# hmakelin/gisnav

Measured on AMD Instinct MI355X. Metric: matched frame-pairs/sec + PnP poses/sec, 640x480 cam-vs-tile, higher is better.
Workload: dtype f32-accurate FFN / out-projection / match-head GEMMs (each f32 operand split into 2 fp16 terms = 22 significant bits, 3 fp16 MFMA partial products, f32 accumulate; fp16-range guard active); attention INPUT projections (q, k, v: 18 of 66 launches) on 2 partial products -- the fp16 high term of the ac

## Files before the change

### gisnav_amd/csrc/gn_api.hip

```cpp
#include "gn_common.h"

#include <cstdio>
#include <cstring>
#include <cmath>
#include <cctype>
#include <algorithm>
#include <tuple>

using namespace gn;

namespace {

thread_local std::string g_err;

struct Linear { float* w = nullptr; float* b = nullptr; int out = 0, in = 0; uint16_t* wp = nullptr; float acc_scale = 1.f;
                uint16_t* wf = nullptr; int frag_order = -1;
                uint16_t* wf2 = nullptr;
                uint16_t* wfn = nullptr; };

struct Block {
  Linear proj_in;
  Linear proj_out;
  Linear ffn0;
  float* ln_g = nullptr; float* ln_b = nullptr;
// ... 93 lines not shown
  float *colbest = nullptr, *col2 = nullptr;
  bool cal_cols = false;
  int precision_api = 0;
  int feature = 0;
  int ransac_iters = 10; float ransac_reproj = 8.0f; double ransac_conf = 0.99;
  gn::PnpArgs last_pnp; bool last_pnp_valid = false; const int32_t* last_npts = nullptr;
  int dist_on = 0; double dist[5] = {0, 0, 0, 0, 0};
  float size_q[2] = {0.f, 0.f}, size_r[2] = {0.f, 0.f};
  int npad_run = 0;
  int n_layers = kMaxLayers;
  float threshold = 0.5f;
  std::string err;
  Linear input_proj;
  float* wr = nullptr;
  Block self_blk[kMaxLayers], cross_blk[kMaxLayers];
  Linear final_proj[kMaxLayers], matchability[kMaxLayers];
  std::map<std::string, bool> loaded;
  std::vector<std::string> required;
  float *desc = nullptr, *cos_t = nullptr, *sin_t = nullptr, *extent = nullptr;
  int32_t* nvalid = nullptr;
  float *x = nullptr, *qkv = nullptr, *ctx = nullptr, *msg = nullptr, *h = nullptr, *md = nullptr, *ls = nullptr;
  uint16_t *desc_p = nullptr, *x_p = nullptr, *ctx_p = nullptr, *msg_p = nullptr, *h_p = nullptr, *md_p = nullptr;
  size_t Tmax = 0;
  int planes_mode = 0;
  float* sim = nullptr;
  uint16_t *qkb = nullptr, *vtb = nullptr;
  float* attn_part = nullptr; unsigned int* attn_tickets = nullptr;
  int attn_split = 1;
  int attn_variant = 4;
  int stop_after = 0;
  int launch_count = 0;
  int no_planes = 0;
  int dbg_planes = 0;
  uint16_t* dbg_wp = nullptr; size_t dbg_wp_n = 0;
  int dbg_out = 0;
  uint16_t* dbg_yp = nullptr; size_t dbg_yp_n = 0;
  int dbg_vt_skip = 0;
  int dbg_reuse = 0;
  uint16_t* dbg_ap = nullptr; size_t dbg_ap_n = 0;
  int gemm_variant = -1;
  float *rowmax = nullptr, *rowlog = nullptr, *colmax = nullptr, *collog = nullptr, *max0 = nullptr;
  int32_t *m0 = nullptr, *m1 = nullptr;
  float *cpart_m = nullptr, *cpart_s = nullptr;
  int32_t* cpart_i = nullptr;
  float* rot4 = nullptr;
  float *rpart_a = nullptr, *rpart_b = nullptr;
  unsigned int* tickets = nullptr;
  int64_t* e_idx = nullptr; float* e_score = nullptr; float* e_mkp = nullptr; float* e_obj = nullptr;
  int defer_join = 0, sub_last_B = 0, sub_last_np = 0;
  int sub_serial = 0;
  int cu_mask_mode = 0;
  int use_lists = 1;
  int ncu = 256;
  int fused_proj_status = -1;
  bool fused_proj_pending = true;
  int fused_proj_off = 0;
  int qkv_in_tail = 1;
  int skinny = 1;
  int auto_level = 3; float cert_eps_lvl[2] = {-1.f, -1.f}; long long auto_pairs = 0, auto_wide = 0, auto_narrow = 0, auto_calls_lvl[2] = {0, 0}, auto_switches = 0;
  int ffn_products = 3;
  int qkv_products = 2;
  unsigned long long* tile_feedback = nullptr;
  int* lists = nullptr; long long lists_stride = 0;
  int n_sub = 1; hipStream_t sub_s[8] = {}; hipEvent_t ev_fork = nullptr; hipEvent_t ev_join[8] = {}; bool sub_pending[8] = {};
  int overlap = 0; unsigned long long calls = 0;
  hipStream_t s_pnp = nullptr; hipEvent_t ev_gather[2][8] = {}, ev_pnp[2][8] = {}; bool pnp_pending[2][8] = {}, pnp_recorded[2][8] = {};
  hipEvent_t ev_head[8] = {};
  float* o_mkp[2] = {nullptr, nullptr}; float* o_obj[2] = {nullptr, nullptr}; int32_t* o_nmatch[2] = {nullptr, nullptr};
  int prep_fused = 1;
  int sift_h = 0, sift_w = 0; std::vector<void*> sift_allocs; SiftPyramid sift_py; float* sift_tmp = nullptr;
  float* sift_dk = nullptr; std::vector<std::vector<float>> sift_kernels; std::vector<int> sift_koff;
  int4* sift_cand = nullptr; int* sift_counts = nullptr; SiftKeypoint* sift_kp = nullptr;
  int sift_max_cand = 0, sift_max_kp = 0, sift_raw_cap = 0, sift_batch = 0; long long sift_kp_stride = 0;
  std::vector<int32_t> sift_totals;
  struct SpConv { float* wf = nullptr; float* b = nullptr; int cout = 0, cin = 0, taps = 0, cout_pad = 0; bool have_w = false, have_b = false;
                  uint16_t* wfh = nullptr; float acc_scale = 1.f; };
  SpConv sp[12];
  std::vector<void*> sp_allocs; int sp_h = 0, sp_w = 0, sp_chunk = 0, sp_cap = 0, sp_max = 0;
  float *sp_x = nullptr, *sp_y = nullptr, *sp_z = nullptr, *sp_maps[6] = {};
  int *sp_cand = nullptr, *sp_counts = nullptr, *sp_index = nullptr;
  float* vo_norm2 = nullptr; int32_t* vo_nn_idx = nullptr; float* vo_nn_dist = nullptr; uint8_t* vo_good = nullptr;
  uint8_t* mask_ws = nullptr;
  float* pts_ws = nullptr;
  gn::HypResult* hyp_ws = nullptr;
  uint8_t* rmask_ws = nullptr;
  gn::RansacState *rstate_ws = nullptr, *rstate_base = nullptr;
  std::vector<void*> allocs;
  std::vector<void*> ws_allocs;
  bool timing = false;
  hipEvent_t ev[2 * 128];
  int ev_stage[128]; int n_ev = 0; bool ev_ready = false;
  float stage_ms[ST_COUNT] = {0};
  bool ktiming = false;
  std::vector<hipEvent_t> kev;
  std::vector<double> kflops;
  std::vector<double> kbytes;
  std::vector<int> kclass;
  std::vector<const char*> kname;
  size_t kused = 0;
};

namespace {

#define GN_HIP(call)                                                                              \
  do {                                                                                            \
    hipError_t e_ = (call);                                                                       \
// ... 362 lines not shown
    StageTimer tm(c, s, ST_PREP);
    PrepArgs p;
    p.desc_q = v.desc_q; p.kpt_q = v.kpt_q; p.n_q = v.n_q; p.stride_q = v.stride_q;
    p.desc_r = v.desc_r; p.kpt_r = v.kpt_r; p.n_r = v.n_r; p.stride_r = v.stride_r;
    p.kpt_format = v.kpt_format; p.B = B; p.npad = np; p.wr = c->wr;
    p.desc = c->desc; p.kxy = nullptr; p.cos_t = c->cos_t; p.sin_t = c->sin_t; p.nvalid = c->nvalid; p.extent = c->extent;
    p.size_q[0] = c->size_q[0]; p.size_q[1] = c->size_q[1]; p.size_r[0] = c->size_r[0]; p.size_r[1] = c->size_r[1];
    p.feature = c->feature; p.x = nullptr; p.xp = nullptr;
    p.ovf_clear = (c->planes_mode && c->guard) ? c->ovf : nullptr;
    p.ovf_init = (c->dbg_trip_group && c->ovf == c->ovf_base + (c->dbg_trip_group - 1)) ? 1u : 0u;
    p.desc_p = nullptr; p.rot4 = nullptr; p.rot_stride = (long long)c->Tmax;
    const bool planes_only = c->planes_mode && c->x_planes_only && c->n_layers > 0;
    if (c->feature == 1) {
      p.x = planes_only ? nullptr : c->x; p.xp = c->planes_mode ? c->x_p : nullptr;
      launch_prep(p, s);
      if (c->rot4 && c->qkv_fused) launch_rot_table(c->cos_t, c->sin_t, c->rot4, T, (long long)c->Tmax, s);
    } else {
      const bool rot = c->rot4 && c->qkv_fused, split = c->planes_mode != 0;
      if (c->prep_fused) { p.rot4 = rot ? c->rot4 : nullptr; p.desc_p = split ? c->desc_p : nullptr; }
      launch_prep(p, s);
      if (rot && !p.rot4) launch_rot_table(c->cos_t, c->sin_t, c->rot4, T, (long long)c->Tmax, s);
      if (split && !p.desc_p) launch_split_hm16(c->desc, c->desc_p, T, kInDim, 1.0f, s);
      GemmArgs g = gemm_args(c->desc, kInDim, c->input_proj, c->x, kDim, T);
      g.drop_f32 = planes_only ? 1 : 0;
      gemm(c, EPI_BIAS, g, s);
    }
  }
  if (c->use_lists && c->lists) {
    const int g = (int)(c->ovf - c->ovf_base);
    launch_tile_lists(c->nvalid, BS, np, c->lists, (c->tile_feedback && g >= 0 && g < 8) ? c->tile_feedback + g : nullptr, s);
  }
  bool qkv_done = false;
  for (int i = 0; i < c->n_layers; ++i) {
    {
      const Block& blk = c->self_blk[i];
      if (!qkv_done) {
        StageTimer tm(c, s, ST_PROJ);
        GemmArgs g = gemm_args(c->x, kDim, blk.proj_in, c->qkv, 3 * kDim, T);
        g.cos_t = c->cos_t; g.sin_t = c->sin_t; g.rot_cols = 2 * kDim;
        if (bf16v2 && qkv_projection(c, blk, false, T, np, vt_perm, s)) {
        } else if (bf16v2) {
          g.Yb = c->qkb; g.ldyb = 2 * kDim; g.Vt = c->vtb; g.vt_start = 2 * kDim; g.q_cols = kDim; g.qscale = 0.125f; g.npad = np; g.vt_perm = vt_perm; g.half_fmt = c->attn_f16;
          gemm(c, EPI_ROTARY_BF16, g, s);
        } else {
          gemm(c, EPI_ROTARY, g, s);
        }
      }
      {
        StageTimer tm(c, s, ST_ATTN);
        AttnArgs a; a.ovf = nullptr;
        a.q = c->qkv; a.ldq = 3 * kDim; a.k = c->qkv + kDim; a.ldk = 3 * kDim; a.v = c->qkv + 2 * kDim; a.ldv = 3 * kDim;
        a.out = c->ctx; a.ldo = kDim; a.nvalid = c->nvalid; a.npad = np; a.cross = 0; a.qscale = 0.125f; a.BS = BS;
        a.outp = attn_planes ? c->ctx_p : nullptr; a.ovf = (attn_planes && c->guard) ? c->ovf : nullptr;
        a.qb = c->qkb; a.ldqb = 2 * kDim; a.kb = c->qkb + kDim; a.ldkb = 2 * kDim; a.vt = c->vtb; a.half_fmt = c->attn_f16; a.tiles = (c->use_lists && c->lists) ? c->lists : nullptr; a.ncu = c->ncu;
        if (bf16v2) attn_split(c, a);
        timed_attention(c, a, bf16v2, s);
        if (c->planes_mode && !attn_planes) launch_split_hm16(c->ctx, c->ctx_p, T, kDim, 1.0f, s);
      }
      if (!tail_folds_out_proj(c, blk, T)) {
        StageTimer tm(c, s, ST_PROJ);
        GemmArgs g = gemm_args(c->ctx, kDim, blk.proj_out, c->msg, kDim, T);
        gemm(c, EPI_BIAS, g, s);
      }
      { StageTimer tm(c, s, ST_FFN); qkv_done = ffn(c, blk, T, s, false, bf16v2 ? &c->cross_blk[i] : nullptr, true, np, vt_perm); }
    }
    {
      const Block& blk = c->cross_blk[i];
      if (!qkv_done) {
        StageTimer tm(c, s, ST_PROJ);
        GemmArgs g = gemm_args(c->x, kDim, blk.proj_in, c->qkv, 2 * kDim, T);
        g.scale = 0.35355339059327373f;
        g.scale_cols = kDim;
        if (bf16v2 && qkv_projection(c, blk, true, T, np, vt_perm, s)) {
        } else if (bf16v2) {
          g.Yb = c->qkb; g.ldyb = kDim; g.Vt = c->vtb; g.vt_start = kDim; g.q_cols = 0; g.qscale = 1.0f; g.npad = np; g.vt_perm = vt_perm; g.half_fmt = c->attn_f16;
          gemm(c, EPI_SCALE_BF16, g, s);
        } else {
          gemm(c, EPI_SCALE_COLS, g, s);
        }
      }
      {
        StageTimer tm(c, s, ST_ATTN);
        AttnArgs a; a.ovf = nullptr;
        a.q = c->qkv; a.ldq = 2 * kDim; a.k = c->qkv; a.ldk = 2 * kDim; a.v = c->qkv + kDim; a.ldv = 2 * kDim;
        a.out = c->ctx; a.ldo = kDim; a.nvalid = c->nvalid; a.npad = np; a.cross = 1; a.qscale = 1.0f; a.BS = BS;
        a.outp = attn_planes ? c->ctx_p : nullptr; a.ovf = (attn_planes && c->guard) ? c->ovf : nullptr;
        a.qb = c->qkb; a.ldqb = kDim; a.kb = c->qkb; a.ldkb = kDim; a.vt = c->vtb; a.half_fmt = c->attn_f16; a.tiles = (c->use_lists && c->lists) ? c->lists : nullptr; a.ncu = c->ncu;
        if (bf16v2) attn_split(c, a);
        timed_attention(c, a, bf16v2, s);
        if (c->planes_mode && !attn_planes) launch_split_hm16(c->ctx, c->ctx_p, T, kDim, 1.0f, s);
      }
      if (!tail_folds_out_proj(c, blk, T)) {
        StageTimer tm(c, s, ST_PROJ);
        GemmArgs g = gemm_args(c->ctx, kDim, blk.proj_out, c->msg, kDim, T);
        gemm(c, EPI_BIAS, g, s);
      }
      { StageTimer tm(c, s, ST_FFN); qkv_done = ffn(c, blk, T, s, i == c->n_layers - 1, (bf16v2 && i + 1 < c->n_layers) ? &c->self_blk[i + 1] : nullptr, false, np, vt_perm); }
    }
  }
  {
    StageTimer tm(c, s, ST_HEAD);
    const int li = c->n_layers - 1;
    GemmArgs g = gemm_args(c->x, kDim, c->final_proj[li], c->md, kDim, T);
    g.scale = 0.25f; g.scale_cols = kDim;
    gemm(c, EPI_SCALE_COLS, g, s);
    launch_matchability(c->x, c->matchability[li].w, c->matchability[li].b, c->ls, T, s);
    HeadArgs hd;
    hd.sim = c->sim; hd.ls = c->ls; hd.nvalid = c->nvalid; hd.B = B; hd.npad = np; hd.threshold = c->threshold;
    hd.rowmax = c->rowmax; hd.rowlog = c->rowlog; hd.colmax = c->colmax; hd.collog = c->collog;
    hd.m0 = c->m0; hd.max0 = c->max0; hd.m1 = c->m1;
    hd.ovf = (c->planes_mode && c->guard) ? c->ovf : nullptr;
    hd.max0b = c->max0b; hd.rpart_c = c->rpart_c; hd.uncert = c->certify ? c->uncert : nullptr;
    hd.cert_eps = (c->precision == GN_PREC_F32) ? c->cert_eps_f32 : cert_eps_now(c);
    if (hd.uncert && c->precision != GN_PREC_F32 && ffn_auto(c)) { hd.uncert_alt = c->uncert_alt; hd.cert_eps_alt = c->cert_eps_lvl[3 - c->auto_level]; }
    hd.idx = v.idx; hd.score = v.score; hd.n_match = v.n_match; hd.kmax = c->npad;
    hd.md = c->planes_mode ? (const void*)c->md_p : (const void*)c->md; hd.md_f32 = c->planes_mode ? 0 : 1;
    hd.cpart_m = c->cpart_m; hd.cpart_s = c->cpart_s; hd.cpart_i = c->cpart_i; hd.rpart_a = c->rpart_a; hd.rpart_b = c->rpart_b; hd.tickets = c->tickets;
    hd.dbg_ts = (c->head_stamps && c->sim) ? reinterpret_cast<long long*>(c->sim) : nullptr;
    if (c->cal_cols) { hd.colbest = c->colbest; hd.col2 = c->col2; }
    if (c->head_fused || !c->sim) {
      timed_launch(c, s, 0, 2.0 * 2.0 * B * (double)np * np * kDim,
                   2.0 * (4.0 * T * kDim) + 4.0 * T * 4.0 + 8.0 * B * np * 3.0,
                   "k_head_fused (2 sweeps)", [&] { launch_match_head_fused(hd, s); });
      return GN_OK;
    }
    GemmArgs gs;
    memset(&gs, 0, sizeof gs);
    gs.A = c->md; gs.lda = kDim; gs.K1 = kDim; gs.W = c->md + (size_t)np * kDim; gs.ldw = kDim;
    gs.Y = c->sim; gs.ldy = np; gs.M = np; gs.N = np; gs.K = kDim; gs.acc_scale = 1.f;
    gs.strideA = gs.strideW = 2LL * np * kDim; gs.strideY = (long long)np * np;
    timed_gemm(c, EPI_PLAIN, gs, B, s);
    launch_match_head(hd, s);
  }
  return GN_OK;
}

int alloc_workspace(gn_ctx* ctx, int max_kpts) {
  ctx->npad = ((max_kpts + 127) / 128) * 128;
  ctx->npad_run = ctx->npad;
  const size_t np = ctx->npad, T = (size_t)ctx->max_batch * 2 * np, B = ctx->max_batch;
// ... 1625 lines not shown
  if (!ctx || !A || !W || !Y || M % 128 || N % 128 || K % 32 || M < 128 || N < 128 || K < 32)
    return fail(ctx, GN_ERR_ARG, "gn_debug_gemm needs M,N multiples of 128 and K a multiple of 32");
  GN_HIP(hipSetDevice(ctx->device));
  GemmArgs g;
  memset(&g, 0, sizeof g);
  g.A = A; g.lda = K; g.K1 = K; g.W = W; g.ldw = K; g.bias = bias; g.Y = Y; g.ldy = N; g.M = M; g.N = N; g.K = K;
  g.acc_scale = 1.f;
  if (ctx->gemm_variant >= 0) gn::g_gemm_variant = ctx->gemm_variant;
  if (ctx->gemm_variant == 7) {
    
    const size_t na = (size_t)M * K, nw = (size_t)N * K;
    if (ctx->dbg_ap_n < na) { ctx->dbg_ap = nullptr; int rc = dalloc(ctx, &ctx->dbg_ap, 2 * na); if (rc != GN_OK) return rc; ctx->dbg_ap_n = na; }
    if (ctx->dbg_wp_n < nw) { ctx->dbg_wp = nullptr; int rc = dalloc(ctx, &ctx->dbg_wp, 3 * nw); if (rc != GN_OK) return rc; ctx->dbg_wp_n = nw; }
    const int e = ctx->dbg_planes > 0 ? ctx->dbg_planes - 1 : 0;
    if (!ctx->dbg_reuse) {
      launch_split_hm16(A, ctx->dbg_ap, M, K, 1.0f, (hipStream_t)stream);
      launch_split_hm16(W, ctx->dbg_wp, N, K, ldexpf(1.0f, e), (hipStream_t)stream);
    }
    g.Ap = ctx->dbg_ap; g.Wp = ctx->dbg_wp; g.acc_scale = ldexpf(1.0f, -e);
    if (ctx->dbg_out) {
      const size_t ny = (size_t)M * N;
      if (ctx->dbg_yp_n < ny) { ctx->dbg_yp = nullptr; int rc = dalloc(ctx, &ctx->dbg_yp, 2 * ny); if (rc != GN_OK) return rc; ctx->dbg_yp_n = ny; }
      g.Yp = ctx->dbg_yp; g.ldyp = N;
      if (ctx->dbg_out == 1) g.Y = nullptr;
    }
    launch_gemm_p2(bias ? EPI_BIAS : EPI_PLAIN, g, 1, (hipStream_t)stream);
    GN_HIP(hipGetLastError());
    return GN_OK;
  }
  if (ctx->dbg_planes) {
    const size_t n = (size_t)N * K;
    if (ctx->dbg_wp_n < n) { ctx->dbg_wp = nullptr; int rc = dalloc(ctx, &ctx->dbg_wp, 3 * n); if (rc != GN_OK) return rc; ctx->dbg_wp_n = n; }
    if (ctx->gemm_variant == 6 || ctx->gemm_variant >= 60) {
      launch_split2_f16(W, ctx->dbg_wp, (long long)n, ldexpf(1.0f, ctx->dbg_planes - 1), (hipStream_t)stream);
      g.acc_scale = ldexpf(1.0f, 1 - ctx->dbg_planes);
    } else {
      launch_split3_bf16(W, ctx->dbg_wp, (long long)n, (hipStream_t)stream);
    }
    g.Wp = ctx->dbg_wp; g.wp_plane = (long long)n;
  }
  launch_gemm_f32(bias ? EPI_BIAS : EPI_PLAIN, g, 1, (hipStream_t)stream);
  GN_HIP(hipGetLastError());
  return GN_OK;
}

int gn_debug_attention(gn_ctx* ctx, int BS, int npad, int cross, float qscale, const float* q, int ldq, const float* k, int ldk,
                       const float* v, int ldv, const int32_t* nkv, float* out, int ldo, void* stream) {
  if (!ctx || !q || !k || !v || !nkv || !out || npad % 128 || BS < 1 || (cross && (BS & 1)))
    return fail(ctx, GN_ERR_ARG, "bad gn_debug_attention argument");
  GN_HIP(hipSetDevice(ctx->device));
  AttnArgs a; a.ovf = nullptr;
  a.q = q; a.ldq = ldq; a.k = k; a.ldk = ldk; a.v = v; a.ldv = ldv; a.out = out; a.ldo = ldo;
  a.nvalid = nkv; a.npad = npad; a.cross = cross; a.qscale = qscale; a.BS = BS;
  a.qb = a.kb = a.vt = nullptr; a.ldqb = a.ldkb = 0; a.outp = nullptr; a.half_fmt = ctx->attn_f16; a.ncu = ctx->ncu;
  const long long cap = (long long)ctx->max_batch * 2 * ctx->npad;
  if (ctx->precision != GN_PREC_F32 && ctx->attn_f16 != 2 && ctx->attn_variant >= 1 && ctx->qkb && ctx->vtb && (long long)BS * npad <= cap) {
    launch_pack_attn_bf16(a, ctx->qkb, ctx->vtb, (hipStream_t)stream);
    a.qb = ctx->qkb; a.kb = ctx->qkb + kDim; a.ldqb = a.ldkb = 2 * kDim; a.vt = ctx->vtb;
    gn::g_attn_variant = ctx->attn_variant;
    gn::g_attn_stamps = (ctx->attn_variant == 73 && ctx->sim) ? reinterpret_cast<long long*>(ctx->sim) : nullptr;
    attn_split(ctx, a);
    launch_attention_bf16_v2(a, (hipStream_t)stream);
  } else {
    attention(ctx, a, (hipStream_t)stream);
  }
  GN_HIP(hipGetLastError());
  return GN_OK;
}

int gn_sp_set_arithmetic(gn_ctx* ctx, int mode) {
  if (!ctx || mode < GN_SP_EXACT_F32 || mode > GN_SP_FP16) return GN_ERR_ARG;
  if (mode != GN_SP_EXACT_F32 && ctx->precision != GN_PREC_F16X2_BF16_ATTN) return fail(ctx, GN_ERR_ARG, "the fp16 SuperPoint arithmetic needs a context of the f16x2 precision");
  ctx->sp_split = mode;
  return GN_OK;
}

static bool retired_variant(int which, int value) {
  switch (which) {
    case 0: return (value >= 51 && value <= 57) || (value >= 61 && value <= 67);
    case 1: return (value >= 41 && value <= 46) || value == 48 || (value >= 51 && value <= 55) || value == 57 || value == 58 ||
                   value == 71 || value == 72 || value >= 1000;
    case 8: return value != 0 && value != 1;
    case 12: return value != 0 && value != 8 && value != 136;
    case 42: return (value & 0xff) != 0;
    default: return false;
  }
}

int gn_debug_set_variant(gn_ctx* ctx, int which, int value) {
  if (!ctx || retired_variant(which, value)) return GN_ERR_ARG;
  if ((which == 1 && value == 73) || (which == 12 && (value & 8)) || (which == 15 && value) || (which == 16 && !value) || (which == 17 && value) || (which == 20 && value)) {
    GN_HIP(hipSetDevice(ctx->device));
    const int rc = ensure_sim(ctx); if (rc != GN_OK) return rc;
  }
  if (which == 0) { gn::g_gemm_variant = value; ctx->gemm_variant = value; }
  else if (which == 1) ctx->attn_variant = value;
  else if (which == 2) ctx->dbg_planes = value;
  else if (which == 3) ctx->no_planes = value;
  else if (which == 4) ctx->stop_after = value;
  else if (which == 5) ctx->planes_mode = (value && ctx->x_p) ? 1 : 0;
  else if (which == 6) ctx->dbg_reuse = value;
  else if (which == 7) ctx->dbg_out = value;
  else if (which == 10) ctx->ffn_fused = value;
  else if (which == 11) ctx->x_planes_only = value;
  else if (which == 8) gn::g_p2_wide = value;
  else if (which == 9) ctx->dbg_vt_skip = value;
  else if (which == 12) gn::g_ffn_stamps = value;
  else if (which == 13) ctx->ffn_fold = value;
  else if (which == 14) gn::g_ffn_shape = value;
  else if (which == 15) ctx->pnp_stamps = value;
  else if (which == 16) ctx->head_fused = value;
  else if (which == 17) ctx->head_stamps = value;
  else if (which == 19) ctx->qkv_fused = value;
  else if (which == 20) ctx->qkv_stamps = value;
  else if (which == 21) ctx->sp_split = value;
  else if (which == 24) gn::g_sp_conv_h = value;
  else if (which == 34) gn::g_sp_conv_s = value;
  else if (which == 36) gn::g_sp_nms_fused = value;
  else if (which == 40) gn::g_sp_select_stream = value;
  else if (which == 41) gn::g_gemm_m64 = value;
  else if (which == 42) gn::g_lf_conv_knob = value;
  else if (which == 43) gn::g_attn_f32_ks = value;
  else if (which == 44) gn::g_gemm_r64 = value;
  else if (which == 46) gn::g_sp_fuse1 = value;
  else if (which == 47) { ctx->fused_proj_pending = value == 0; }
  else if (which == 39) ctx->sp_stop = value;
  else if (which == 35) {
    ctx->sp_ts_layer = value;
    if (value > 0 && ctx->sp_ts == nullptr) { void* q = nullptr; if (hipMalloc(&q, (size_t)8192 * 32 * sizeof(long long)) == hipSuccess) { ctx->sp_ts = (long long*)q; ctx->sp_allocs_dbg = q; } }
    if (ctx->sp_ts != nullptr) hipMemset(ctx->sp_ts, 0, (size_t)8192 * 32 * sizeof(long long));
  }
  else if (which == 23) ctx->attn_split = value;
  else if (which == 25) ctx->dbg_trip_group = value;
  else if (which == 26) ctx->sub_serial = value;
  else if (which == 27) ctx->qkv_products = value == 3 ? 3 : 2;
  else if (which == 28) ctx->ffn_compose = value;
  else if (which == 31) ctx->use_lists = value;
  else if (which == 32) ctx->qkv_in_tail = value ? 1 : 0;
  else if (which == 33) ctx->skinny = value;
  else if (which == 48) ctx->prep_fused = value ? 1 : 0;
  else if (which == 49) ctx->pnp_rounds = value ? 1 : 0;
  else if (which == 29) {
    GN_HIP(hipSetDevice(ctx->device));
    for (int i = 0; i < 8; ++i) if (ctx->sub_s[i]) { hipStreamSynchronize(ctx->sub_s[i]); hipEventDestroy(ctx->ev_join[i]); hipStreamDestroy(ctx->sub_s[i]); ctx->sub_s[i] = nullptr; ctx->ev_join[i] = nullptr; }
    ctx->cu_mask_mode = value;
    if (ctx->n_sub > 1) { const int n = ctx->n_sub; ctx->n_sub = 1; return gn_set_substreams(ctx, n); }
  }
  else return GN_ERR_ARG;
  return GN_OK;
}

int gn_debug_epnp(gn_ctx* ctx, int n, const double* pws, const double* us, double* out, void* stream) {
  if (!ctx || n < 1 || !pws || !us || !out) return GN_ERR_ARG;
  GN_HIP(hipSetDevice(ctx->device));
  launch_epnp_debug(pws, us, out, n, (hipStream_t)stream);
  GN_HIP(hipGetLastError());
  return GN_OK;
}

int gn_debug_lds_dma_probe(gn_ctx* ctx, const float* pattern, unsigned int* out, int blocks, int spin, void* stream) {
  if (!ctx || !pattern || !out || blocks < 1) return GN_ERR_ARG;
  GN_HIP(hipSetDevice(ctx->device));
  launch_lds_dma_probe(pattern, out, blocks, spin, (hipStream_t)stream);
  GN_HIP(hipGetLastError());
  return GN_OK;
}

int gn_debug_mfma_probe(gn_ctx* ctx, int blocks, int iters, void* stream) {
  if (!ctx || blocks < 1 || iters == 0) return GN_ERR_ARG;
  GN_HIP(hipSetDevice(ctx->device));
  launch_mfma_probe(ctx->ls, blocks, iters, (hipStream_t)stream);
  GN_HIP(hipGetLastError());
  return GN_OK;
}

int gn_set_kernel_timing(gn_ctx* ctx, int max_launches) {
  if (!ctx || max_launches < 0) return GN_ERR_ARG;
  hipSetDevice(ctx->device);
  while ((int)ctx->kflops.size() < max_launches) {
    hipEvent_t a, b;
    if (hipEventCreate(&a) != hipSuccess || hipEventCreate(&b) != hipSuccess) return GN_ERR_HIP;
    ctx->kev.push_back(a); ctx->kev.push_back(b); ctx->kflops.push_back(0.0); ctx->kbytes.push_back(0.0); ctx->kclass.push_back(0); ctx->kname.push_back("");
  }
  ctx->ktiming = max_launches > 0;
  ctx->kused = 0;
  return GN_OK;
}

int gn_get_kernel_stats(gn_ctx* ctx, int kernel_class, double* out3) {
  if (!ctx || !out3 || kernel_class < 0 || kernel_class > 1) return GN_ERR_ARG;
  hipSetDevice(ctx->device);
  double ms = 0.0, fl = 0.0, n = 0.0;
  for (size_t i = 0; i < ctx->kused; ++i) {
    if (hipEventSynchronize(ctx->kev[2 * i + 1]) != hipSuccess) return GN_ERR_HIP;
// ... 69 lines not shown
```

### gisnav_amd/csrc/gn_attention_pw.hip

```cpp
#include "gn_common.h"
#include <type_traits>

namespace gn {

namespace {
constexpr int KT = 64;
constexpr float kLog2e = 1.4426950408889634f;
constexpr int kRing = 64 * 64;
constexpr int kSlabPitch = 272;
typedef __attribute__((address_space(3))) void* lptr_t;
typedef unsigned int u32x4 __attribute__((ext_vector_type(4)));
#define GN_PIN() __builtin_amdgcn_sched_barrier(0)

template <bool F16> __device__ __forceinline__ f32x16 mfma16(const bf16x8& x, const bf16x8& y, const f32x16& c) {
  if constexpr (F16) {
    typedef _Float16 f16x8_t __attribute__((ext_vector_type(8)));
    return __builtin_amdgcn_mfma_f32_32x32x16_f16(__builtin_bit_cast(f16x8_t, x), __builtin_bit_cast(f16x8_t, y), c, 0, 0, 0);
  } else {
    return __builtin_amdgcn_mfma_f32_32x32x16_bf16(x, y, c, 0, 0, 0);
  }
}
template <bool F16> __device__ __forceinline__ void mfma_v0(f32x16& s, const bf16x8& x, const bf16x8& y) {
  if constexpr (F16) asm volatile("v_mfma_f32_32x32x16_f16 %0, %1, %2, 0" : "=&v"(s) : "v"(x), "v"(y));
  else asm volatile("v_mfma_f32_32x32x16_bf16 %0, %1, %2, 0" : "=&v"(s) : "v"(x), "v"(y));
}
template <bool F16> __device__ __forceinline__ void mfma_v(f32x16& s, const bf16x8& x, const bf16x8& y) {
  if constexpr (F16) asm volatile("v_mfma_f32_32x32x16_f16 %0, %1, %2, %0" : "+v"(s) : "v"(x), "v"(y));
  else asm volatile("v_mfma_f32_32x32x16_bf16 %0, %1, %2, %0" : "+v"(s) : "v"(x), "v"(y));
}

template <bool F16, int ABL>
__global__ __launch_bounds__(256) void k_attn_pw(AttnArgs a, int nitems) {
  constexpr int NDK = 4, NDV = 3, NW = 4, NQ = 2, IPW = 8 / NW;
  __shared__ __attribute__((aligned(1024))) unsigned short smem[(NDK + NDV) * kRing + NW * 32 * kSlabPitch / 2];
  const int gx = a.npad / (NW * 32 * NQ);
  const int n_work = a.tiles != nullptr ? a.tiles[1] : nitems;
  const int first = (int)(blockIdx.x & 7) * ((int)gridDim.x >> 3) + ((int)blockIdx.x >> 3);
#pragma unroll 1
  for (int work = first; work < n_work; work += gridDim.x) {
  int tid = threadIdx.x;
  asm volatile("" : "+v"(tid));
  const int lane = tid & 63, wave = tid >> 6;
  const int hh = lane >> 5, ql = lane & 31;
  int qblk, h, bs;
  {
    const int v = a.tiles != nullptr ? a.tiles[kTileListBase + a.BS * (a.npad / 128) + work] : work;
    qblk = v % gx;
    const int g = v / gx;
    h = g % kHeads; bs = g / kHeads;
  }
  long long ts[8];
  auto stamp = [&](int k) __attribute__((always_inline)) { if (ABL & 8) ts[k] = (long long)__builtin_amdgcn_s_memtime(); };
  stamp(0);
  const int kvs = a.cross ? (bs ^ 1) : bs;
  const int q0 = qblk * (NW * 32 * NQ) + wave * 32 * NQ;

  const int wave_u = __builtin_amdgcn_readfirstlane(wave);
  unsigned kvo[IPW], vvo[IPW];
  const unsigned short* kbase[IPW]; const unsigned short* vbase[IPW];
#pragma unroll
  for (int j = 0; j < IPW; ++j) {
    const int r0 = (IPW * wave_u + j) * 8, r = r0 + (lane >> 3);
    const int c = (lane & 7) ^ ((r ^ (r >> 3)) & 7);
    kvo[j] = (unsigned)(((lane >> 3) * a.ldkb + c * 8) * 2);
    vvo[j] = (unsigned)(((lane >> 3) * a.npad + c * 8) * 2);
    kbase[j] = a.kb + ((size_t)kvs * a.npad + r0) * a.ldkb + h * 64;
    vbase[j] = a.vt + (((size_t)kvs * kHeads + h) * kHeadDim + r0) * a.npad;
  }
  const size_t kstep = (size_t)KT * a.ldkb;
  const unsigned lds0 = (unsigned)(size_t)(lptr_t)smem;
  auto dma16 = [&](unsigned voff, const unsigned short* sbase, unsigned lds_byte) __attribute__((always_inline)) {
    asm volatile("s_mov_b32 m0, %2\n\ts_nop 0\n\tglobal_load_lds_dwordx4 %0, %1" ::"v"(voff), "s"(sbase), "s"(lds_byte) : "memory");
  };
#define GN_DMA_K(stage, t)                                                                                              \
  _Pragma("unroll") for (int j = 0; j < IPW; ++j)                                                                       \
    dma16(kvo[j], kbase[j] + (size_t)(t) * kstep, lds0 + 2 * ((stage) * kRing + (IPW * wave_u + j) * 512));
#define GN_DMA_V(stage, t)                                                                                              \
  _Pragma("unroll") for (int j = 0; j < IPW; ++j)                                                                       \
    dma16(vvo[j], vbase[j] + (t) * KT, lds0 + 2 * ((NDK + (stage)) * kRing + (IPW * wave_u + j) * 512));

  GN_DMA_K(0, 0);
  GN_DMA_K(1, 1); GN_DMA_V(0, 0);
  GN_DMA_K(2, 2); GN_DMA_V(1, 1);
  const int nkv = a.nvalid[kvs];
  const int ntiles = (nkv + KT - 1) / KT;
  bf16x8 qf[NQ][4];
#pragma unroll
  for (int qi = 0; qi < NQ; ++qi) {
    const unsigned short* qp = a.qb + ((size_t)bs * a.npad + q0 + 32 * qi + ql) * a.ldqb + h * 64 + 8 * hh;
#pragma unroll
    for (int c = 0; c < 4; ++c) qf[qi][c] = *reinterpret_cast<const bf16x8*>(qp + 16 * c);
  }
  f32x16 o[NQ][2], ol[NQ];
#pragma unroll
  for (int qi = 0; qi < NQ; ++qi)
#pragma unroll
    for (int r = 0; r < 16; ++r) { o[qi][0][r] = 0.f; o[qi][1][r] = 0.f; ol[qi][r] = 0.f; }
  bf16x8 ones;
#pragma unroll
  for (int e = 0; e < 8; ++e) ones[e] = (short)(F16 ? 0x3c00 : 0x3f80);
  float m_run[NQ] = {-INFINITY, -INFINITY}, mneg[NQ] = {0.f, 0.f};

  unsigned kfo[2][4], vfo[2][2][2];
#pragma unroll
  for (int i2 = 0; i2 < 2; ++i2) {
    const int row = i2 * 32 + ql, f = (row ^ (row >> 3)) & 7;
#pragma unroll
    for (int c = 0; c < 4; ++c) kfo[i2][c] = (unsigned)(row * 128 + (((2 * c + hh) ^ f) << 4));
#pragma unroll
    for (int kt = 0; kt < 2; ++kt)
#pragma unroll
      for (int u = 0; u < 2; ++u) vfo[i2][kt][u] = (unsigned)(row * 128 + (((4 * kt + 2 * u + hh) ^ f) << 4));
  }
  const unsigned char* const lds = reinterpret_cast<const unsigned char*>(smem);
  auto k_frag = [&](unsigned stage_byte, int kt, int c) __attribute__((always_inline)) {
    return *reinterpret_cast<const bf16x8*>(lds + (stage_byte + kfo[kt][c]));
  };
  auto v_frag = [&](unsigned stage_byte, int d, int kt, int u) __attribute__((always_inline)) {
    return *reinterpret_cast<const bf16x8*>(lds + (stage_byte + vfo[d][kt][u]));
  };

  f32x16 Sa[NQ], Sb[NQ];
  bf16x8 pf[NQ][2];
  float mloc[NQ];
  bool grow = false;

  float mt[NQ][5];
  auto m_step = [&](f32x16 (&S)[NQ], int qi, int st, int key0, auto mask_tag) __attribute__((always_inline)) {
    if (st == 0) {
      if constexpr (decltype(mask_tag)::value) {
        const int lim = nkv - key0 - 4 * hh;
#pragma unroll
        for (int r = 0; r < 16; ++r)
          if ((r & 3) + 8 * (r >> 2) >= lim) S[qi][r] = -INFINITY;
      }
#pragma unroll
      for (int i = 0; i < 5; ++i) mt[qi][i] = __builtin_fmaxf(__builtin_fmaxf(S[qi][3 * i], S[qi][3 * i + 1]), S[qi][3 * i + 2]);
    } else if (st == 1) {
      const float x = __builtin_fmaxf(__builtin_fmaxf(mt[qi][0], mt[qi][1]), mt[qi][2]);
      const float y = __builtin_fmaxf(__builtin_fmaxf(mt[qi][3], mt[qi][4]), S[qi][15]);
      mloc[qi] = __builtin_fmaxf(x, y);
    } else {
      grow = grow || (mloc[qi] - m_run[qi]) * kLog2e > 8.0f;
    }
  };
// ... 52 lines not shown
    kf[1] = k_frag(0, 1, 1);
  }
  stamp(2);

  auto subtile = [&](const f32x16 (&SC)[NQ], f32x16 (&SN)[NQ], unsigned kst, int ktn, unsigned kst2, int kt2, unsigned vst, int kt, int next_key0,
                     auto mask, bool live) __attribute__((always_inline)) {
    bf16x8 vf[2][2];
#pragma unroll
    for (int c = 0; c < 4; ++c) {
#pragma unroll
      for (int qi = 0; qi < NQ; ++qi) {
        const int m = 2 * c + qi;
        if (c == 0) mfma_v0<F16>(SN[qi], kf[c % 3], qf[qi][c]); else mfma_v<F16>(SN[qi], kf[c % 3], qf[qi][c]);
#pragma unroll
        for (int st = (10 * m) / 8; st < (10 * (m + 1)) / 8; ++st) e_step(SC, st / 5, st % 5);
        if (qi == 0) {
          __builtin_amdgcn_sched_barrier(0);
          if (c < 2) kf[(c + 2) % 3] = k_frag(kst, ktn, c + 2);
          vf[c & 1][c >> 1] = v_frag(vst, c & 1, kt, c >> 1);
        }
        GN_PIN();
      }
    }
#pragma unroll
    for (int u = 0; u < 2; ++u) {
#pragma unroll
      for (int i = 0; i < 6; ++i) {
        const int qi = i & 1, m = 6 * u + i;
        if (u == 1 && i == 0) kf[0] = k_frag(kst2, kt2, 0);
        if (u == 1 && i == 2) kf[1] = k_frag(kst2, kt2, 1);
        if (i < 2) ol[qi] = mfma16<F16>(ones, pf[qi][u], ol[qi]);
        else o[qi][(i - 2) >> 1] = mfma16<F16>(vf[(i - 2) >> 1][u], pf[qi][u], o[qi][(i - 2) >> 1]);
        if (m < 6) {
#pragma unroll
          for (int st = (10 * m) / 6; st < (10 * (m + 1)) / 6; ++st) e_step(SC, 2 + st / 5, st % 5);
        } else {
          const int mm = m - 6;
          if (mm < 2) m_step(SN, mm, 0, next_key0, mask);
          else if (mm == 2) { m_step(SN, 0, 1, next_key0, mask); m_step(SN, 1, 1, next_key0, mask); }
          else if (mm == 3) { m_step(SN, 0, 2, next_key0, mask); m_step(SN, 1, 2, next_key0, mask); }
        }
        GN_PIN();
      }
    }
    asm volatile("" ::"v"(SN[0]), "v"(SN[1]));
    if (live) rescale(); else grow = false;
  };

  int k0 = 0, k1 = 1, k2 = 2, k3 = 3;
  int v0 = 0, v1 = 1, v2 = 2;
  auto tile = [&](int t, auto mask_a, auto mask_b) __attribute__((always_inline)) {
    if (t + 2 < ntiles) asm volatile("s_waitcnt vmcnt(4) lgkmcnt(0)\n\ts_barrier" ::: "memory");
    else asm volatile("s_waitcnt vmcnt(0) lgkmcnt(0)\n\ts_barrier" ::: "memory");
    if (t + 3 < ntiles) GN_DMA_K(k3, t + 3);
    if (t + 2 < ntiles) GN_DMA_V(v2, t + 2);
    const unsigned ks0 = 2 * kRing * k0, ks1 = 2 * kRing * k1, vs0 = 2 * kRing * (NDK + v0);
    GN_PIN();
    subtile(Sa, Sb, ks0, 1, ks1, 0, vs0, 0, t * KT + 32, mask_a, true);
    subtile(Sb, Sa, ks1, 0, ks1, 1, vs0, 1, t * KT + 64, mask_b, t + 1 < ntiles);
    { const int s_ = k0; k0 = k1; k1 = k2; k2 = k3; k3 = s_; }
    { const int s_ = v0; v0 = v1; v1 = v2; v2 = s_; }
  };
#pragma unroll 1
  for (int t = 0; t + 2 < ntiles; ++t) tile(t, std::false_type{}, std::false_type{});
  if (ntiles >= 2) tile(ntiles - 2, std::false_type{}, std::true_type{});
  if (ntiles >= 1) tile(ntiles - 1, std::true_type{}, std::false_type{});
  stamp(3);
  stamp(4);
#undef GN_DMA_K
#undef GN_DMA_V

  if (a.outp != nullptr) {
    typedef _Float16 f16x4 __attribute__((ext_vector_type(4)));
    typedef float f32x4v __attribute__((ext_vector_type(4)));
    unsigned char* const slab = reinterpret_cast<unsigned char*>(smem) + 2 * (NDK + NDV) * kRing + wave * 32 * kSlabPitch;
    const int nq = a.nvalid[bs];
    float amax = 0.f;
#pragma unroll
    for (int qi = 0; qi < NQ; ++qi) {
      const float l = ol[qi][0];
      const float inv = l > 0.f ? 1.0f / l : 0.f;
      float amq = 0.f;
#pragma unroll
      for (int d = 0; d < 2; ++d)
#pragma unroll
        for (int g = 0; g < 4; ++g) {
          const f32x4v w = {o[qi][d][4 * g + 0] * inv, o[qi][d][4 * g + 1] * inv, o[qi][d][4 * g + 2] * inv, o[qi][d][4 * g + 3] * inv};
          ovf_track(amq, w.x, w.y); ovf_track(amq, w.z, w.w);
          const f16x4 hv = __builtin_convertvector(w, f16x4);
          const f16x4 mv = __builtin_convertvector(w - __builtin_convertvector(hv, f32x4v), f16x4);
          unsigned char* pp = slab + ql * kSlabPitch + (2 * d + (g >> 1)) * 64 + (8 * (g & 1) + 4 * hh) * 2;
          *reinterpret_cast<f16x4*>(pp) = hv;
          *reinterpret_cast<f16x4*>(pp + 32) = mv;
        }
      if (q0 + 32 * qi + ql < nq) amax = fmaxf(amax, amq);
#pragma unroll
      for (int j = 0; j < 8; ++j) {
        const int row = 4 * j + (lane >> 4), ch = lane & 15;
        const uint4 val = *reinterpret_cast<const uint4*>(slab + row * kSlabPitch + ch * 16);
        uint16_t* dst = a.outp + hm16_off((size_t)bs * a.npad + q0 + 32 * qi + row, a.ldo, h * 64) + ch * 8;
        *reinterpret_cast<uint4*>(dst) = val;
      }
    }
    ovf_commit(a.ovf, amax);
  } else {
#pragma unroll
    for (int qi = 0; qi < NQ; ++qi) {
      const float l = ol[qi][0];
      const float inv = l > 0.f ? 1.0f / l : 0.f;
      float* op = a.out + ((size_t)bs * a.npad + q0 + 32 * qi + ql) * a.ldo + h * 64 + 4 * hh;
#pragma unroll
      for (int d = 0; d < 2; ++d)
#pragma unroll
        for (int g = 0; g < 4; ++g) {
          float4 w;
          w.x = o[qi][d][4 * g + 0] * inv; w.y = o[qi][d][4 * g + 1] * inv;
          w.z = o[qi][d][4 * g + 2] * inv; w.w = o[qi][d][4 * g + 3] * inv;
          *reinterpret_cast<float4*>(op + d * 32 + 8 * g) = w;
        }
    }
  }
  asm volatile("s_waitcnt lgkmcnt(0)\n\ts_barrier" ::: "memory");
  if (ABL & 8) {
    asm volatile("s_waitcnt vmcnt(0)" ::: "memory");
    stamp(5);
    if (lane == 0) {
      long long* dst = reinterpret_cast<long long*>(a.part) + ((size_t)(blockIdx.x + gridDim.x * (blockIdx.y + gridDim.y * blockIdx.z)) * NW + wave) * 8;
      for (int k = 0; k < 6; ++k) dst[k] = ts[k];
      dst[6] = ntiles; dst[7] = 0;
    }
  }
  }
}
#undef GN_PIN
}

bool launch_attention_pw(const AttnArgs& a, bool stamps, hipStream_t s) {
  if (a.npad % 256 != 0 || a.qb == nullptr) return false;
  const int nitems = a.npad / 256 * kHeads * a.BS;
  if (nitems < 8) return false;
  const int ncu = a.ncu >= 8 ? a.ncu : std::max(device_cu_count(), 8);
  const dim3 grid((unsigned)((stamps || nitems < ncu) ? (nitems & ~7) : (ncu & ~7))), block(256);
  if (a.half_fmt) {
    if (stamps) {
      if (g_attn_stamps == nullptr) return false;
      AttnArgs b = a; b.part = reinterpret_cast<float*>(g_attn_stamps); b.tiles = nullptr;
      hipLaunchKernelGGL((k_attn_pw<true, 8>), grid, block, 0, s, b, nitems);
    }
    else hipLaunchKernelGGL((k_attn_pw<true, 0>), grid, block, 0, s, a, nitems);
    g_last_kernel = "k_attn_pw<true, 0>";
  } else {
    hipLaunchKernelGGL((k_attn_pw<false, 0>), grid, block, 0, s, a, nitems);
    g_last_kernel = "k_attn_pw<false, 0>";
  }
  return true;
}

}
```

### gisnav_amd/csrc/gn_common.h

```cpp
#pragma once
#include <hip/hip_runtime.h>
#include <stdint.h>
#include <string>
#include <vector>
#include <map>

#include "../../include/gisnav_amd.h"

namespace gn {

constexpr int kDim = 256;
constexpr int kHeads = 4;
constexpr int kHeadDim = 64;
constexpr int kInDim = 128;
constexpr int kFreq = 32;
constexpr int kMaxLayers = 9;
constexpr int kRecordFloats = 133;

typedef float f32x4 __attribute__((ext_vector_type(4)));
typedef float f32x16 __attribute__((ext_vector_type(16)));
typedef short bf16x8 __attribute__((ext_vector_type(8)));

__device__ __forceinline__ float gelu_erf(float y) {
  const float t = fminf(fabsf(y) * 0.70710678118654752440f, 4.0f);
// ... 119 lines not shown
  unsigned int* ovf;
  long long* dbg_ts;
  const int* tiles = nullptr;
  int products = 2;
  int ncu = 0;
};
void launch_qkv(const QkvArgs& a, bool cross, hipStream_t s);
void launch_skinny_qkv(const QkvArgs& a, bool cross, hipStream_t s);
struct SkinnyTailArgs {
  const uint16_t* xp = nullptr; const uint16_t* cp = nullptr;
  const uint16_t* w1 = nullptr; float w1_scale = 1.f; const float* b1 = nullptr;
  float* h = nullptr;
  const float* ln_g = nullptr; const float* ln_b = nullptr;
  const uint16_t* w2 = nullptr; float w2_scale = 1.f; const float* b2 = nullptr;
  uint16_t* xp_out = nullptr; float* y = nullptr;
  unsigned int* ovf = nullptr; int T = 0;
};
void launch_skinny_h(const SkinnyTailArgs& a, hipStream_t s, int variant = 0);
void launch_skinny_out(const SkinnyTailArgs& a, hipStream_t s, int variant = 0);
int device_cu_count();

struct AttnArgs {
  const uint16_t* qb; int ldqb;
  const uint16_t* kb; int ldkb;
  const uint16_t* vt;
  const float* q; int ldq;
  const float* k; int ldk;
  const float* v; int ldv;
  float* out; int ldo;
  uint16_t* outp;
  const int32_t* nvalid;
  int npad;
  int cross;
  float qscale;
  int BS;
  unsigned int* ovf;
  int half_fmt = 0;
  int nsplit = 1;
  float* part = nullptr;
  unsigned int* tickets = nullptr;
  const int* tiles = nullptr;
  int ncu = 0;
};
constexpr int kTileListBase = 16;
void launch_tile_lists(const int32_t* nvalid, int BS, int npad, int* lists, unsigned long long* feedback , hipStream_t s);
void launch_attention_f32(const AttnArgs& a, hipStream_t s);
void launch_attention_bf16(const AttnArgs& a, hipStream_t s);
void launch_attention_f16x2(const AttnArgs& a, hipStream_t s);
void launch_attention_bf16_v2(const AttnArgs& a, hipStream_t s);
bool launch_attention_pw(const AttnArgs& a, bool stamps, hipStream_t s);
void launch_pack_attn_bf16(const AttnArgs& a, uint16_t* qkb, uint16_t* vtb, hipStream_t s);
extern thread_local long long* g_attn_stamps;
extern thread_local int g_attn_variant;

struct PrepArgs {
  const float* desc_q; const float* kpt_q; const int32_t* n_q; int stride_q;
  const float* desc_r; const float* kpt_r; const int32_t* n_r; int stride_r;
  int kpt_format; int B; int npad;
  const float* wr;
  float* desc;
  float* kxy;
  float* cos_t; float* sin_t;
  int32_t* nvalid;
  float* extent;
  float size_q[2], size_r[2];
  int feature;
  float* x; uint16_t* xp;
  uint16_t* desc_p;
  float* rot4; long long rot_stride;
  unsigned int* ovf_clear; unsigned int ovf_init;
};
void launch_prep(const PrepArgs& a, hipStream_t s);
void launch_ln_gelu(float* h, const float* gamma, const float* beta, int rows, hipStream_t s,
                    uint16_t* hp = nullptr, unsigned int* ovf = nullptr);
void launch_matchability(const float* x, const float* w, const float* b, float* ls, int rows, hipStream_t s);

struct HeadArgs {
  const float* sim;
  const float* ls;
  const int32_t* nvalid;
  int B; int npad; float threshold;
  float* rowmax; float* rowlog; float* colmax; float* collog;
  int32_t* m0; float* max0; int32_t* m1;
  int64_t* idx; float* score; int32_t* n_match; int kmax;
  const unsigned int* ovf;
  const void* md;
  int md_f32;
  float* cpart_m; float* cpart_s; int32_t* cpart_i;
  float* rpart_a; float* rpart_b;
  unsigned int* tickets;
  long long* dbg_ts;
  float* max0b;
  float* rpart_c;
  int32_t* uncert;
  float cert_eps;
  int32_t* uncert_alt = nullptr;
  float cert_eps_alt = -1.f;
  float* colbest = nullptr;
  float* col2 = nullptr;
};
void launch_match_head(const HeadArgs& a, hipStream_t s);
void launch_match_head_fused(const HeadArgs& a, hipStream_t s);

struct GatherArgs {
  const float* kpt_q; int stride_q; const float* kpt_r; int stride_r; int kpt_format;
  const int64_t* idx; const int32_t* n_match; int kmax; int B;
// ... 116 lines not shown
```

Baseline: 5823.

## Prefetch next attention work item's K/V and Q during current item's epilogue

In the persistent attention kernel, the DMA of the next work item's first K/V tiles and its Q fragments is issued before the current item's output epilogue. This hides the start-up latency at the seam between items, and the trailing barrier is skipped when a prefetch is already in flight. Two knobs are also added: one selects the old non-seamed variant and one caps the attention grid size. The cost is longer register live ranges for the next item's Q fragments, plus an added ordering constraint on the shared-memory ring between the epilogue and the new DMA.

```diff
diff --git a/gisnav_amd/csrc/gn_api.hip b/gisnav_amd/csrc/gn_api.hip
--- a/gisnav_amd/csrc/gn_api.hip
+++ b/gisnav_amd/csrc/gn_api.hip
@@ -169,6 +169,7 @@
   int cu_mask_mode = 0;
   int use_lists = 1;
   int ncu = 256;
+  int attn_grid_cap = 0;
   int fused_proj_status = -1;
   bool fused_proj_pending = true;
   int fused_proj_off = 0;
@@ -637,7 +638,7 @@
         a.q = c->qkv; a.ldq = 3 * kDim; a.k = c->qkv + kDim; a.ldk = 3 * kDim; a.v = c->qkv + 2 * kDim; a.ldv = 3 * kDim;
         a.out = c->ctx; a.ldo = kDim; a.nvalid = c->nvalid; a.npad = np; a.cross = 0; a.qscale = 0.125f; a.BS = BS;
         a.outp = attn_planes ? c->ctx_p : nullptr; a.ovf = (attn_planes && c->guard) ? c->ovf : nullptr;
-        a.qb = c->qkb; a.ldqb = 2 * kDim; a.kb = c->qkb + kDim; a.ldkb = 2 * kDim; a.vt = c->vtb; a.half_fmt = c->attn_f16; a.tiles = (c->use_lists && c->lists) ? c->lists : nullptr; a.ncu = c->ncu;
+        a.qb = c->qkb; a.ldqb = 2 * kDim; a.kb = c->qkb + kDim; a.ldkb = 2 * kDim; a.vt = c->vtb; a.half_fmt = c->attn_f16; a.tiles = (c->use_lists && c->lists) ? c->lists : nullptr; a.ncu = c->attn_grid_cap ? c->attn_grid_cap : c->ncu;
         if (bf16v2) attn_split(c, a);
         timed_attention(c, a, bf16v2, s);
         if (c->planes_mode && !attn_planes) launch_split_hm16(c->ctx, c->ctx_p, T, kDim, 1.0f, s);
@@ -670,7 +671,7 @@
         a.q = c->qkv; a.ldq = 2 * kDim; a.k = c->qkv; a.ldk = 2 * kDim; a.v = c->qkv + kDim; a.ldv = 2 * kDim;
         a.out = c->ctx; a.ldo = kDim; a.nvalid = c->nvalid; a.npad = np; a.cross = 1; a.qscale = 1.0f; a.BS = BS;
         a.outp = attn_planes ? c->ctx_p : nullptr; a.ovf = (attn_planes && c->guard) ? c->ovf : nullptr;
-        a.qb = c->qkb; a.ldqb = kDim; a.kb = c->qkb; a.ldkb = kDim; a.vt = c->vtb; a.half_fmt = c->attn_f16; a.tiles = (c->use_lists && c->lists) ? c->lists : nullptr; a.ncu = c->ncu;
+        a.qb = c->qkb; a.ldqb = kDim; a.kb = c->qkb; a.ldkb = kDim; a.vt = c->vtb; a.half_fmt = c->attn_f16; a.tiles = (c->use_lists && c->lists) ? c->lists : nullptr; a.ncu = c->attn_grid_cap ? c->attn_grid_cap : c->ncu;
         if (bf16v2) attn_split(c, a);
         timed_attention(c, a, bf16v2, s);
         if (c->planes_mode && !attn_planes) launch_split_hm16(c->ctx, c->ctx_p, T, kDim, 1.0f, s);
@@ -2402,7 +2403,7 @@
   AttnArgs a; a.ovf = nullptr;
   a.q = q; a.ldq = ldq; a.k = k; a.ldk = ldk; a.v = v; a.ldv = ldv; a.out = out; a.ldo = ldo;
   a.nvalid = nkv; a.npad = npad; a.cross = cross; a.qscale = qscale; a.BS = BS;
-  a.qb = a.kb = a.vt = nullptr; a.ldqb = a.ldkb = 0; a.outp = nullptr; a.half_fmt = ctx->attn_f16; a.ncu = ctx->ncu;
+  a.qb = a.kb = a.vt = nullptr; a.ldqb = a.ldkb = 0; a.outp = nullptr; a.half_fmt = ctx->attn_f16; a.ncu = ctx->attn_grid_cap ? ctx->attn_grid_cap : ctx->ncu;
   const long long cap = (long long)ctx->max_batch * 2 * ctx->npad;
   if (ctx->precision != GN_PREC_F32 && ctx->attn_f16 != 2 && ctx->attn_variant >= 1 && ctx->qkb && ctx->vtb && (long long)BS * npad <= cap) {
     launch_pack_attn_bf16(a, ctx->qkb, ctx->vtb, (hipStream_t)stream);
@@ -2490,6 +2491,8 @@
   else if (which == 33) ctx->skinny = value;
   else if (which == 48) ctx->prep_fused = value ? 1 : 0;
   else if (which == 49) ctx->pnp_rounds = value ? 1 : 0;
+  else if (which == 50) gn::g_attn_pw_noseam = value ? 1 : 0;
+  else if (which == 51) { if (value < 0 || (value & 7)) return GN_ERR_ARG; ctx->attn_grid_cap = value; }
   else if (which == 29) {
     GN_HIP(hipSetDevice(ctx->device));
     for (int i = 0; i < 8; ++i) if (ctx->sub_s[i]) { hipStreamSynchronize(ctx->sub_s[i]); hipEventDestroy(ctx->ev_join[i]); hipStreamDestroy(ctx->sub_s[i]); ctx->sub_s[i] = nullptr; ctx->ev_join[i] = nullptr; }
diff --git a/gisnav_amd/csrc/gn_attention_pw.hip b/gisnav_amd/csrc/gn_attention_pw.hip
--- a/gisnav_amd/csrc/gn_attention_pw.hip
+++ b/gisnav_amd/csrc/gn_attention_pw.hip
@@ -29,13 +29,77 @@
   else asm volatile("v_mfma_f32_32x32x16_bf16 %0, %1, %2, %0" : "+v"(s) : "v"(x), "v"(y));
 }
 
+template <int IPW> struct DmaAddr {
+  unsigned kvo[IPW], vvo[IPW];
+  const unsigned short* kbase[IPW]; const unsigned short* vbase[IPW];
+};
+
 template <bool F16, int ABL>
 __global__ __launch_bounds__(256) void k_attn_pw(AttnArgs a, int nitems) {
   constexpr int NDK = 4, NDV = 3, NW = 4, NQ = 2, IPW = 8 / NW;
+  constexpr bool SEAM = ABL == 0;
   __shared__ __attribute__((aligned(1024))) unsigned short smem[(NDK + NDV) * kRing + NW * 32 * kSlabPitch / 2];
   const int gx = a.npad / (NW * 32 * NQ);
   const int n_work = a.tiles != nullptr ? a.tiles[1] : nitems;
   const int first = (int)(blockIdx.x & 7) * ((int)gridDim.x >> 3) + ((int)blockIdx.x >> 3);
+  auto item_word = [&](int w) __attribute__((always_inline)) {
+    return a.tiles != nullptr ? a.tiles[kTileListBase + a.BS * (a.npad / 128) + w] : w;
+  };
+  auto decode = [&](int v, int& qblk, int& h, int& bs) __attribute__((always_inline)) {
+    qblk = v % gx;
+    const int g = v / gx;
+    h = g % kHeads; bs = g / kHeads;
+  };
+  auto dma_addr = [&](DmaAddr<IPW>& d, int lane, int wave_u, int kvs, int h) __attribute__((always_inline)) {
+#pragma unroll
+    for (int j = 0; j < IPW; ++j) {
+      const int r0 = (IPW * wave_u + j) * 8, r = r0 + (lane >> 3);
+      const int c = (lane & 7) ^ ((r ^ (r >> 3)) & 7);
+      d.kvo[j] = (unsigned)(((lane >> 3) * a.ldkb + c * 8) * 2);
+      d.vvo[j] = (unsigned)(((lane >> 3) * a.npad + c * 8) * 2);
+      d.kbase[j] = a.kb + ((size_t)kvs * a.npad + r0) * a.ldkb + h * 64;
+      d.vbase[j] = a.vt + (((size_t)kvs * kHeads + h) * kHeadDim + r0) * a.npad;
+    }
+  };
+  const size_t kstep = (size_t)KT * a.ldkb;
+  const unsigned lds0 = (unsigned)(size_t)(lptr_t)smem;
+  auto dma16 = [&](unsigned voff, const unsigned short* sbase, unsigned lds_byte) __attribute__((always_inline)) {
+    asm volatile("s_mov_b32 m0, %2\n\ts_nop 0\n\tglobal_load_lds_dwordx4 %0, %1" ::"v"(voff), "s"(sbase), "s"(lds_byte) : "memory");
+  };
+#define GN_DMA_K(d, wu, stage, t)                                                                                       \
+  _Pragma("unroll") for (int j = 0; j < IPW; ++j)                                                                       \
+    dma16((d).kvo[j], (d).kbase[j] + (size_t)(t) * kstep, lds0 + 2 * ((stage) * kRing + (IPW * (wu) + j) * 512));
+#define GN_DMA_V(d, wu, stage, t)                                                                                       \
+  _Pragma("unroll") for (int j = 0; j < IPW; ++j)                                                                       \
+    dma16((d).vvo[j], (d).vbase[j] + (t) * KT, lds0 + 2 * ((NDK + (stage)) * kRing + (IPW * (wu) + j) * 512));
+  bf16x8 qf[NQ][4];
+  auto request = [&](const DmaAddr<IPW>& d, int wave_u, int qblk, int h, int bs, int wave, int ql, int hh) __attribute__((always_inline)) {
+    GN_DMA_K(d, wave_u, 0, 0);
+    GN_DMA_K(d, wave_u, 1, 1); GN_DMA_V(d, wave_u, 0, 0);
+    GN_DMA_K(d, wave_u, 2, 2); GN_DMA_V(d, wave_u, 1, 1);
+    const int q0 = qblk * (NW * 32 * NQ) + wave * 32 * NQ;
+#pragma unroll
+    for (int qi = 0; qi < NQ; ++qi) {
+      const unsigned short* qp = a.qb + ((size_t)bs * a.npad + q0 + 32 * qi + ql) * a.ldqb + h * 64 + 8 * hh;
+#pragma unroll
+      for (int c = 0; c < 4; ++c) qf[qi][c] = *reinterpret_cast<const bf16x8*>(qp + 16 * c);
+    }
+  };
+  auto request_item = [&](int w) __attribute__((always_inline)) {
+    int tid = threadIdx.x;
+    asm volatile("" : "+v"(tid));
+    const int lane = tid & 63, wave = tid >> 6;
+    const int v = __builtin_amdgcn_readfirstlane(item_word(w));
+    int qblk, h, bs;
+    decode(v, qblk, h, bs);
+    DmaAddr<IPW> d;
+    const int wave_u = __builtin_amdgcn_readfirstlane(wave);
+    dma_addr(d, lane, wave_u, a.cross ? (bs ^ 1) : bs, h);
+    request(d, wave_u, qblk, h, bs, wave, lane & 31, lane >> 5);
+    return v;
+  };
+  int v_item = 0;
+  if (SEAM && first < n_work) v_item = request_item(first);
 #pragma unroll 1
   for (int work = first; work < n_work; work += gridDim.x) {
   int tid = threadIdx.x;
@@ -43,12 +107,7 @@
   const int lane = tid & 63, wave = tid >> 6;
   const int hh = lane >> 5, ql = lane & 31;
   int qblk, h, bs;
-  {
-    const int v = a.tiles != nullptr ? a.tiles[kTileListBase + a.BS * (a.npad / 128) + work] : work;
-    qblk = v % gx;
-    const int g = v / gx;
-    h = g % kHeads; bs = g / kHeads;
-  }
+  decode(SEAM ? v_item : item_word(work), qblk, h, bs);
   long long ts[8];
   auto stamp = [&](int k) __attribute__((always_inline)) { if (ABL & 8) ts[k] = (long long)__builtin_amdgcn_s_memtime(); };
   stamp(0);
@@ -56,41 +115,12 @@
   const int q0 = qblk * (NW * 32 * NQ) + wave * 32 * NQ;
 
   const int wave_u = __builtin_amdgcn_readfirstlane(wave);
-  unsigned kvo[IPW], vvo[IPW];
-  const unsigned short* kbase[IPW]; const unsigned short* vbase[IPW];
-#pragma unroll
-  for (int j = 0; j < IPW; ++j) {
-    const int r0 = (IPW * wave_u + j) * 8, r = r0 + (lane >> 3);
-    const int c = (lane & 7) ^ ((r ^ (r >> 3)) & 7);
-    kvo[j] = (unsigned)(((lane >> 3) * a.ldkb + c * 8) * 2);
-    vvo[j] = (unsigned)(((lane >> 3) * a.npad + c * 8) * 2);
-    kbase[j] = a.kb + ((size_t)kvs * a.npad + r0) * a.ldkb + h * 64;
-    vbase[j] = a.vt + (((size_t)kvs * kHeads + h) * kHeadDim + r0) * a.npad;
-  }
-  const size_t kstep = (size_t)KT * a.ldkb;
-  const unsigned lds0 = (unsigned)(size_t)(lptr_t)smem;
-  auto dma16 = [&](unsigned voff, const unsigned short* sbase, unsigned lds_byte) __attribute__((always_inline)) {
-    asm volatile("s_mov_b32 m0, %2\n\ts_nop 0\n\tglobal_load_lds_dwordx4 %0, %1" ::"v"(voff), "s"(sbase), "s"(lds_byte) : "memory");
-  };
-#define GN_DMA_K(stage, t)                                                                                              \
-  _Pragma("unroll") for (int j = 0; j < IPW; ++j)                                                                       \
-    dma16(kvo[j], kbase[j] + (size_t)(t) * kstep, lds0 + 2 * ((stage) * kRing + (IPW * wave_u + j) * 512));
-#define GN_DMA_V(stage, t)                                                                                              \
-  _Pragma("unroll") for (int j = 0; j < IPW; ++j)                                                                       \
-    dma16(vvo[j], vbase[j] + (t) * KT, lds0 + 2 * ((NDK + (stage)) * kRing + (IPW * wave_u + j) * 512));
-
-  GN_DMA_K(0, 0);
-  GN_DMA_K(1, 1); GN_DMA_V(0, 0);
-  GN_DMA_K(2, 2); GN_DMA_V(1, 1);
+  DmaAddr<IPW> da;
+  dma_addr(da, lane, wave_u, kvs, h);
+  if constexpr (!SEAM) request(da, wave_u, qblk, h, bs, wave, ql, hh);
   const int nkv = a.nvalid[kvs];
   const int ntiles = (nkv + KT - 1) / KT;
-  bf16x8 qf[NQ][4];
-#pragma unroll
-  for (int qi = 0; qi < NQ; ++qi) {
-    const unsigned short* qp = a.qb + ((size_t)bs * a.npad + q0 + 32 * qi + ql) * a.ldqb + h * 64 + 8 * hh;
-#pragma unroll
-    for (int c = 0; c < 4; ++c) qf[qi][c] = *reinterpret_cast<const bf16x8*>(qp + 16 * c);
-  }
+  const int nq = __builtin_amdgcn_readfirstlane(a.nvalid[bs]);
   f32x16 o[NQ][2], ol[NQ];
 #pragma unroll
   for (int qi = 0; qi < NQ; ++qi)
@@ -249,8 +279,8 @@
   auto tile = [&](int t, auto mask_a, auto mask_b) __attribute__((always_inline)) {
     if (t + 2 < ntiles) asm volatile("s_waitcnt vmcnt(4) lgkmcnt(0)\n\ts_barrier" ::: "memory");
     else asm volatile("s_waitcnt vmcnt(0) lgkmcnt(0)\n\ts_barrier" ::: "memory");
-    if (t + 3 < ntiles) GN_DMA_K(k3, t + 3);
-    if (t + 2 < ntiles) GN_DMA_V(v2, t + 2);
+    if (t + 3 < ntiles) GN_DMA_K(da, wave_u, k3, t + 3);
+    if (t + 2 < ntiles) GN_DMA_V(da, wave_u, v2, t + 2);
     const unsigned ks0 = 2 * kRing * k0, ks1 = 2 * kRing * k1, vs0 = 2 * kRing * (NDK + v0);
     GN_PIN();
     subtile(Sa, Sb, ks0, 1, ks1, 0, vs0, 0, t * KT + 32, mask_a, true);
@@ -264,14 +294,20 @@
   if (ntiles >= 1) tile(ntiles - 1, std::true_type{}, std::false_type{});
   stamp(3);
   stamp(4);
-#undef GN_DMA_K
-#undef GN_DMA_V
+
+  bool more = false;
+  if constexpr (SEAM) {
+    more = work + (int)gridDim.x < n_work;
+    if (more) {
+      asm volatile("s_waitcnt lgkmcnt(0)\n\ts_barrier" ::: "memory");
+      v_item = request_item(work + (int)gridDim.x);
+    }
+  }
 
   if (a.outp != nullptr) {
     typedef _Float16 f16x4 __attribute__((ext_vector_type(4)));
     typedef float f32x4v __attribute__((ext_vector_type(4)));
     unsigned char* const slab = reinterpret_cast<unsigned char*>(smem) + 2 * (NDK + NDV) * kRing + wave * 32 * kSlabPitch;
-    const int nq = a.nvalid[bs];
     float amax = 0.f;
 #pragma unroll
     for (int qi = 0; qi < NQ; ++qi) {
@@ -317,7 +353,7 @@
         }
     }
   }
-  asm volatile("s_waitcnt lgkmcnt(0)\n\ts_barrier" ::: "memory");
+  if (!more) asm volatile("s_waitcnt lgkmcnt(0)\n\ts_barrier" ::: "memory");
   if (ABL & 8) {
     asm volatile("s_waitcnt vmcnt(0)" ::: "memory");
     stamp(5);
@@ -328,9 +364,13 @@
     }
   }
   }
+#undef GN_DMA_K
+#undef GN_DMA_V
 }
 #undef GN_PIN
 }
+
+int g_attn_pw_noseam = 0;
 
 bool launch_attention_pw(const AttnArgs& a, bool stamps, hipStream_t s) {
   if (a.npad % 256 != 0 || a.qb == nullptr) return false;
@@ -344,11 +384,13 @@
       AttnArgs b = a; b.part = reinterpret_cast<float*>(g_attn_stamps); b.tiles = nullptr;
       hipLaunchKernelGGL((k_attn_pw<true, 8>), grid, block, 0, s, b, nitems);
     }
+    else if (g_attn_pw_noseam) hipLaunchKernelGGL((k_attn_pw<true, 4>), grid, block, 0, s, a, nitems);
     else hipLaunchKernelGGL((k_attn_pw<true, 0>), grid, block, 0, s, a, nitems);
-    g_last_kernel = "k_attn_pw<true, 0>";
+    g_last_kernel = (g_attn_pw_noseam && !stamps) ? "k_attn_pw<true, 4>" : "k_attn_pw<true, 0>";
   } else {
-    hipLaunchKernelGGL((k_attn_pw<false, 0>), grid, block, 0, s, a, nitems);
-    g_last_kernel = "k_attn_pw<false, 0>";
+    if (g_attn_pw_noseam) hipLaunchKernelGGL((k_attn_pw<false, 4>), grid, block, 0, s, a, nitems);
+    else hipLaunchKernelGGL((k_attn_pw<false, 0>), grid, block, 0, s, a, nitems);
+    g_last_kernel = g_attn_pw_noseam ? "k_attn_pw<false, 4>" : "k_attn_pw<false, 0>";
   }
   return true;
 }
diff --git a/gisnav_amd/csrc/gn_common.h b/gisnav_amd/csrc/gn_common.h
--- a/gisnav_amd/csrc/gn_common.h
+++ b/gisnav_amd/csrc/gn_common.h
@@ -195,6 +195,7 @@
 void launch_pack_attn_bf16(const AttnArgs& a, uint16_t* qkb, uint16_t* vtb, hipStream_t s);
 extern thread_local long long* g_attn_stamps;
 extern thread_local int g_attn_variant;
+extern int g_attn_pw_noseam;
 
 struct PrepArgs {
   const float* desc_q; const float* kpt_q; const int32_t* n_q; int stride_q;
```

After: 5850 (median of 6 runs). No clear change (+0.5%).
